# xrouting/xroute_env

Measured on AMD Instinct MI355X. Metric: env-steps/sec (batched regions), ispd18_test1-sized regions, higher is better.
Workload: dtype u32 distances / i16 state / fp32 observation

## Files before the change

xroute_env_amd/csrc/xr_kernels.hip:

```cpp
#include <hip/hip_runtime.h>
#include <stdint.h>
#include <initializer_list>
#include <type_traits>

#include "xr_device.h"
#include "../../include/xroute_hip.h"

#define XR_FNV_PRIME 0x100000001b3ULL

__device__ __forceinline__ void fnv_mix(uint64_t& h, uint32_t w) { h = (h ^ (uint64_t)w) * XR_FNV_PRIME; }

__device__ __forceinline__ uint64_t splitmix64(uint64_t x) {
    x += 0x9E3779B97F4A7C15ULL;
    uint64_t z = x;
    z = (z ^ (z >> 30)) * 0xBF58476D1CE4E5B9ULL;
    z = (z ^ (z >> 27)) * 0x94D049BB133111EBULL;
    return z ^ (z >> 31);
}

__global__ void xr_ingest_kernel(const uint32_t* __restrict__ rec, int16_t* __restrict__ node_net,
                                 int16_t* __restrict__ owner0, int64_t total) {
    int64_t i = (int64_t)blockIdx.x * blockDim.x + threadIdx.x;
    const int64_t stride = (int64_t)gridDim.x * blockDim.x;
    for (; i < total; i += stride) {
// ... 717 lines not shown
    const uint64_t* lw = b.legal + (int64_t)row * b.legal_words;
    int act = 0;
    for (int w = 0; w < b.legal_words; w++) {
        uint64_t m = lw[w];
        const int pc = __popcll(m);
        if (j >= pc) { j -= pc; continue; }
        while (j > 0) { m &= m - 1; j--; }
        act = w * 64 + __ffsll((long long)m);
        break;
    }
    return act;
}

__global__ void xr_random_action_kernel(XrBatchDev b, int32_t* __restrict__ actions, uint64_t seed) {
    const int e = b.env_base + blockIdx.x * blockDim.x + threadIdx.x;
    if (e >= XR_ENV_END(b)) return;
    actions[e] = xr_random_pick(b, e, e, seed);
}

struct XrStateSrc {
    const int16_t* node_net;
    const int16_t* owner;
    __device__ __forceinline__ int net(int f) const { const int n = node_net[f]; return n; }
    __device__ __forceinline__ bool used(int f) const { return owner[f] != 0; }
};
struct XrRecSrc {
    const uint32_t* rec;
    __device__ __forceinline__ int net(int f) const {
        const uint32_t r = rec[f];
        const uint32_t t = XR_REC_TYPE(r);
        return t == XR_TYPE_ACCESS ? (int)XR_REC_NET1(r) : (t == XR_TYPE_BLOCKAGE ? -1 : 0);
    }
    __device__ __forceinline__ bool used(int f) const { return XR_REC_USED(rec[f]) != 0; }
};

template <class Src>
__device__ __forceinline__ void xr_node_features(const Src& s, int f, int X, int Y, int Z, int N, float& obst,
                                                 int& apnet, bool& adj) {
    if (f >= N) { obst = 0.f; apnet = 0; adj = false; return; }
    const int n = s.net(f);
    const bool used = s.used(f);
    obst = (n == -1 || used) ? 1.f : 0.f;
    apnet = n > 0 ? n : 0;
    adj = false;
    if (n > 0) {
        const int z = f % Z, y = (f / Z) % Y, x = f / (Y * Z);
        const int YZ = Y * Z;
        if (x + 1 < X && s.net(f + YZ) == n) adj = true;
        else if (y > 0 && s.net(f - Z) == n) adj = true;
        else if (x > 0 && s.net(f - YZ) == n) adj = true;
        else if (y + 1 < Y && s.net(f + Z) == n) adj = true;
        else if (z + 1 < Z && s.net(f + 1) == n) adj = true;
        else if (z > 0 && s.net(f - 1) == n) adj = true;
    }
}

typedef float xr_f4 __attribute__((ext_vector_type(4)));
#define XR_ST4(ptr, val) __builtin_nontemporal_store(xr_f4{(val).x, (val).y, (val).z, (val).w}, reinterpret_cast<xr_f4*>(ptr))
template <class Src, int VEC>
__device__ __forceinline__ void xr_obs_write(const Src& s, int X, int Y, int Z, int N, const int* s_ids, int K,
                                             float* __restrict__ out, int chunk_base, int knets = -1) {
    if (knets < 0) knets = K;
    const int f0 = chunk_base + threadIdx.x * VEC;
    if (f0 >= N) return;
    float obst[VEC];
    int apnet[VEC];
    bool adj[VEC];
#pragma unroll
    for (int j = 0; j < VEC; j++) xr_node_features(s, f0 + j, X, Y, Z, N, obst[j], apnet[j], adj[j]);
    float* p = out + f0;
    if (VEC == 4) {
        float4 v;
        v.x = obst[0]; v.y = obst[1]; v.z = obst[2]; v.w = obst[3];
        XR_ST4(p, v);
        p += N;
        v.x = (f0 + 0 < K) ? (float)s_ids[f0 + 0] : 0.f;
        v.y = (f0 + 1 < K) ? (float)s_ids[f0 + 1] : 0.f;
        v.z = (f0 + 2 < K) ? (float)s_ids[f0 + 2] : 0.f;
        v.w = (f0 + 3 < K) ? (float)s_ids[f0 + 3] : 0.f;
        XR_ST4(p, v);
        p += N;
        bool anyap = false;
#pragma unroll
        for (int j = 0; j < VEC; j++) anyap |= (apnet[j] != 0);
        const float4 zero = make_float4(0.f, 0.f, 0.f, 0.f);
        for (int i = 0; i < knets; i++) {
            float4 m = zero, ma = zero;
            if (anyap) {
                const int id = s_ids[i];
                m.x = (apnet[0] == id) ? 1.f : 0.f; m.y = (apnet[1] == id) ? 1.f : 0.f;
                m.z = (apnet[2] == id) ? 1.f : 0.f; m.w = (apnet[3] == id) ? 1.f : 0.f;
                ma.x = (adj[0] ? m.x : 0.f); ma.y = (adj[1] ? m.y : 0.f);
                ma.z = (adj[2] ? m.z : 0.f); ma.w = (adj[3] ? m.w : 0.f);
            }
            XR_ST4(p, m);
            p += N;
#pragma unroll
            for (int c = 0; c < 6; c++) { XR_ST4(p, ma); p += N; }
        }
    } else {
        p[0] = obst[0];
        p += N;
        p[0] = (f0 < K) ? (float)s_ids[f0] : 0.f;
        p += N;
        for (int i = 0; i < knets; i++) {
            const float m = (apnet[0] != 0 && apnet[0] == s_ids[i]) ? 1.f : 0.f;
            const float ma = adj[0] ? m : 0.f;
            p[0] = m;
            p += N;
#pragma unroll
            for (int c = 0; c < 6; c++) { p[0] = ma; p += N; }
        }
    }
}

__device__ __forceinline__ float xr_plane_value(unsigned ft, int plane, int node, const int* s_ids, int K) {
    if (plane >= 2) {
        const int pi = plane - 2, i = pi / 7, c = pi - 7 * i;
        const unsigned id = (unsigned)s_ids[i];
        return c ? (((ft & 0x7FFFu) == (id | 0x4000u)) ? 1.f : 0.f) : (((ft & 0x3FFFu) == id) ? 1.f : 0.f);
    }
    if (plane == 0) return (ft & 0x8000u) ? 1.f : 0.f;
    return node < K ? (float)s_ids[node] : 0.f;
}

template <class Src>
__device__ __forceinline__ void xr_obs_env_stream(const Src& src, int X, int Y, int Z, int N, const int* s_ids, int K,
                                                  float* __restrict__ out, unsigned short* s_feat, int planes = -1) {
    const int tid = threadIdx.x, nthr = blockDim.x;
#pragma unroll 4
    for (int f = tid; f < N; f += nthr) {
        float obst; int apnet; bool adj;
        xr_node_features(src, f, X, Y, Z, N, obst, apnet, adj);
        s_feat[f] = (unsigned short)(apnet | (adj ? 0x4000 : 0) | (obst != 0.f ? 0x8000 : 0));
    }
    __syncthreads();
    const long long total = (long long)(planes >= 0 ? planes : 2 + 7 * K) * N;
    const long long nslot = total >> 2;
    int plane = (int)((4LL * tid) / N), node = (int)((4LL * tid) - (long long)plane * N);
    const int dplane = (4 * nthr) / N, dnode = (4 * nthr) - dplane * N;
    for (long long sidx = tid; sidx < nslot; sidx += nthr) {
        float v[4];
        if (node + 3 < N && plane >= 2) {
            const int pi = plane - 2, i = pi / 7, c = pi - 7 * i;
            const unsigned id = (unsigned)s_ids[i];
            const unsigned msk = c ? 0x7FFFu : 0x3FFFu, want = c ? (id | 0x4000u) : id;
#pragma unroll
            for (int j = 0; j < 4; j++) v[j] = ((s_feat[node + j] & msk) == want) ? 1.f : 0.f;
        } else {
            int p = plane, f = node;
#pragma unroll
            for (int j = 0; j < 4; j++) {
                v[j] = xr_plane_value(s_feat[f], p, f, s_ids, K);
                if (++f == N) { f = 0; ++p; }
            }
        }
        XR_ST4(out + 4 * sidx, make_float4(v[0], v[1], v[2], v[3]));
        plane += dplane; node += dnode;
        if (node >= N) { node -= N; ++plane; }
    }
    const int tail = (int)(total & 3);
    if (tid < tail) {
        const long long g = (nslot << 2) + tid;
        const int p = (int)(g / N), f = (int)(g - (long long)p * N);
        out[g] = xr_plane_value(s_feat[f], p, f, s_ids, K);
    }
}

__device__ __forceinline__ int xr_legal_ids_pre(uint64_t my_m, int words, int* s_ids, int* s_pref) {
    const int tid = threadIdx.x;
    if (tid < words) s_pref[tid] = __popcll(my_m);
    xr_lds_barrier();
    if (tid == 0) {
        int acc = 0;
        for (int w = 0; w < words; w++) { const int c = s_pref[w]; s_pref[w] = acc; acc += c; }
        s_pref[words] = acc;
    }
    xr_lds_barrier();
    if (tid < words) {
        uint64_t m = my_m;
        int o = s_pref[tid];
        while (m) { const int bit = __ffsll((long long)m) - 1; s_ids[o++] = tid * 64 + bit + 1; m &= m - 1; }
    }
    xr_lds_barrier();
    return s_pref[words];
}
__device__ __forceinline__ int xr_legal_ids(const uint64_t* __restrict__ lw, int words, int* s_ids, int* s_pref) {
    const int tid = threadIdx.x;
    for (int w = tid; w < words; w += blockDim.x) s_pref[w] = __popcll(lw[w]);
    __syncthreads();
    if (tid == 0) {
        int acc = 0;
        for (int w = 0; w < words; w++) { const int c = s_pref[w]; s_pref[w] = acc; acc += c; }
        s_pref[words] = acc;
    }
    __syncthreads();
    for (int w = tid; w < words; w += blockDim.x) {
        uint64_t m = lw[w];
        int o = s_pref[w];
        while (m) { const int bit = __ffsll((long long)m) - 1; s_ids[o++] = w * 64 + bit + 1; m &= m - 1; }
    }
    __syncthreads();
    return s_pref[words];
}

template <int VEC>
__global__ void xr_obs_kernel(XrBatchDev b, float* __restrict__ out, int64_t env_stride, int env_lo) {
    extern __shared__ __attribute__((aligned(16))) char smem[];
    int* s_ids = reinterpret_cast<int*>(smem);
    int* s_pref = s_ids + b.legal_words * 64;
    const int e = env_lo + blockIdx.y;
    const XrRegionDev R = b.regions[b.env_region[e]];
    const int chunk_base = blockIdx.x * blockDim.x * VEC;
    if (chunk_base >= R.N) return;
    const int K = xr_legal_ids(b.legal + (int64_t)e * b.legal_words, b.legal_words, s_ids, s_pref);
    XrStateSrc src{b.rg_node_net + R.node_off, b.owner + (int64_t)e * b.n_max};
    xr_obs_write<XrStateSrc, VEC>(src, R.X, R.Y, R.Z, R.N, s_ids, K, out + (int64_t)blockIdx.y * env_stride,
                                  chunk_base);
}

__global__ void xr_obs_stream_kernel(XrBatchDev b, float* __restrict__ out, int64_t env_stride, int env_lo) {
    extern __shared__ __attribute__((aligned(16))) char smem[];
    int* s_ids = reinterpret_cast<int*>(smem);
    int* s_pref = s_ids + b.legal_words * 64;
    unsigned short* s_feat = reinterpret_cast<unsigned short*>(s_pref + ((b.legal_words + 1 + 3) & ~3));
    const int e = env_lo + blockIdx.x;
    const XrRegionDev R = b.regions[b.env_region[e]];
    const int K = xr_legal_ids(b.legal + (int64_t)e * b.legal_words, b.legal_words, s_ids, s_pref);
    XrStateSrc src{b.rg_node_net + R.node_off, b.owner + (int64_t)e * b.n_max};
    xr_obs_env_stream(src, R.X, R.Y, R.Z, R.N, s_ids, K, out + (int64_t)blockIdx.x * env_stride, s_feat);
}

template <int VEC>
__global__ void xr_obs_records_kernel(const uint32_t* __restrict__ rec, int X, int Y, int Z,
                                      const int32_t* __restrict__ nets, int K, float* __restrict__ out) {
    extern __shared__ __attribute__((aligned(16))) char smem[];
    int* s_ids = reinterpret_cast<int*>(smem);
    for (int i = threadIdx.x; i < K; i += blockDim.x) s_ids[i] = nets[i];
    __syncthreads();
    XrRecSrc src{rec};
    xr_obs_write<XrRecSrc, VEC>(src, X, Y, Z, X * Y * Z, s_ids, K, out, blockIdx.x * blockDim.x * VEC);
}

__device__ __forceinline__ void xr_obs_epilogue(const XrBatchDev& b, int e, char* smem, bool head_only) {
    __syncthreads();
    const XrRegionDev R = b.regions[b.env_region[e]];
    int* s_ids = reinterpret_cast<int*>(smem);
    int* s_pref = s_ids + b.legal_words * 64;
    XrStateSrc src{b.rg_node_net + R.node_off, b.owner + (int64_t)e * b.n_max};
    float* __restrict__ out = b.obs_out + (int64_t)e * b.obs_stride;
    const int ids_bytes = ((b.legal_words * 64 + b.legal_words + 1) * 4 + 15) & ~15;
    const int npad = (R.N + 7) & ~7;
    if (b.obs_vec4 == 1 && ids_bytes + 4 * npad <= b.obs_lds_bytes && b.legal_words <= (int)blockDim.x) {
        const int tid = threadIdx.x, nthr = (int)blockDim.x;
        const uint64_t my_m = tid < b.legal_words ? b.legal[(int64_t)e * b.legal_words + tid] : 0ull;
        int16_t* l_nn = reinterpret_cast<int16_t*>(smem + ids_bytes);
        int16_t* l_ow = l_nn + npad;
        const int nchunk = npad >> 3;
#pragma unroll 4
        for (int ci = tid; ci < nchunk; ci += nthr) {
            const int4 vn = *reinterpret_cast<const int4*>(src.node_net + (ci << 3));
            const int4 vo = *reinterpret_cast<const int4*>(src.owner + (ci << 3));
            *reinterpret_cast<int4*>(l_nn + (ci << 3)) = vn;
            *reinterpret_cast<int4*>(l_ow + (ci << 3)) = vo;
        }
        const int K = xr_legal_ids_pre(my_m, b.legal_words, s_ids, s_pref);
        const int knets = head_only ? XR_SPLIT_KEEP(b, K) : K;
        XrStateSrc lsrc{l_nn, l_ow};
        for (int cb = 0; cb < R.N; cb += nthr * 4)
            xr_obs_write<XrStateSrc, 4>(lsrc, R.X, R.Y, R.Z, R.N, s_ids, K, out, cb, knets);
        return;
    }
    const int feat_bytes = (b.legal_words * 64 + ((b.legal_words + 1 + 3) & ~3)) * 4;
    if (b.obs_vec4 == 2 && feat_bytes + 4 * npad <= b.obs_lds_bytes && b.legal_words <= (int)blockDim.x) {
        const int tid = threadIdx.x, nthr = (int)blockDim.x;
        const uint64_t my_m = tid < b.legal_words ? b.legal[(int64_t)e * b.legal_words + tid] : 0ull;
        unsigned short* s_feat = reinterpret_cast<unsigned short*>(smem + feat_bytes);
        int16_t* l_nn = reinterpret_cast<int16_t*>(smem + feat_bytes + 2 * npad);
        const int nchunk = npad >> 3;
#pragma unroll 4
        for (int ci = tid; ci < nchunk; ci += nthr)
            *reinterpret_cast<int4*>(l_nn + (ci << 3)) = *reinterpret_cast<const int4*>(src.node_net + (ci << 3));
        const int K = xr_legal_ids_pre(my_m, b.legal_words, s_ids, s_pref);
        XrStateSrc lsrc{l_nn, src.owner};
        const int planes = head_only ? 2 + 7 * XR_SPLIT_KEEP(b, K) : -1;
        xr_obs_env_stream(lsrc, R.X, R.Y, R.Z, R.N, s_ids, K, out, s_feat, planes);
        return;
    }
    const int K = xr_legal_ids(b.legal + (int64_t)e * b.legal_words, b.legal_words, s_ids, s_pref);
    if (b.obs_vec4 == 1) {
        const int knets = head_only ? XR_SPLIT_KEEP(b, K) : K;
        for (int cb = 0; cb < R.N; cb += (int)blockDim.x * 4)
            xr_obs_write<XrStateSrc, 4>(src, R.X, R.Y, R.Z, R.N, s_ids, K, out, cb, knets);
    } else if (b.obs_vec4 == 2) {
        unsigned short* s_feat = reinterpret_cast<unsigned short*>(s_pref + ((b.legal_words + 1 + 3) & ~3));
        const int planes = head_only ? 2 + 7 * XR_SPLIT_KEEP(b, K) : -1;
        xr_obs_env_stream(src, R.X, R.Y, R.Z, R.N, s_ids, K, out, s_feat, planes);
    } else {
        for (int cb = 0; cb < R.N; cb += (int)blockDim.x)
            xr_obs_write<XrStateSrc, 1>(src, R.X, R.Y, R.Z, R.N, s_ids, K, out, cb);
    }
}

__device__ __forceinline__ int xr_route_work_class(const XrBatchDev& b, const int32_t* __restrict__ actions, int e) {
    const int a = actions[e];
    const XrRegionDev& R = b.regions[b.env_region[e]];
    if (a < 1 || a > R.n_nets || b.done[e]) return 0;
    if (!((b.legal[(int64_t)e * b.legal_words + ((a - 1) >> 6)] >> ((a - 1) & 63)) & 1ull)) return 0;
    if (b.net_meas) { const int m = b.net_meas[R.net_off + a]; if (m) return m; }
    return b.net_work[R.net_off + a];
}

__global__ void __launch_bounds__(1024) xr_route_order_kernel(XrBatchDev b, const int32_t* __restrict__ actions, int32_t* __restrict__ order) {
    __shared__ uint32_t s_cnt[256];
    __shared__ uint32_t s_wsum[4];
    const int t = threadIdx.x;
    if (t < 256) s_cnt[t] = 0;
    __syncthreads();
    const int e0 = b.env_base, e1 = XR_ENV_END(b);
    int cls[8];
#pragma unroll
    for (int k = 0; k < 8; k++) {
        const int e = e0 + t + k * 1024;
        cls[k] = e < e1 ? xr_route_work_class(b, actions, e) : -1;
        if (cls[k] >= 0) atomicAdd(&s_cnt[cls[k]], 1u);
    }
    for (int e = e0 + t + 8 * 1024; e < e1; e += 1024) atomicAdd(&s_cnt[xr_route_work_class(b, actions, e)], 1u);
    __syncthreads();
    uint32_t v = 0, incl = 0;
    if (t < 256) {
        v = s_cnt[255 - t];
        incl = v;
        for (int o = 1; o < 64; o <<= 1) {
            const uint32_t u = __shfl_up(incl, o, 64);
            if ((t & 63) >= o) incl += u;
        }
        if ((t & 63) == 63) s_wsum[t >> 6] = incl;
    }
    __syncthreads();
    if (t < 256) {
        uint32_t base = 0;
        for (int w = 0; w < (t >> 6); w++) base += s_wsum[w];
        s_cnt[255 - t] = base + incl - v;
    }
    __syncthreads();
#pragma unroll
    for (int k = 0; k < 8; k++)
        if (cls[k] >= 0) order[atomicAdd(&s_cnt[cls[k]], 1u)] = e0 + t + k * 1024;
    for (int e = e0 + t + 8 * 1024; e < e1; e += 1024) order[atomicAdd(&s_cnt[xr_route_work_class(b, actions, e)], 1u)] = e;
}

template <bool LDS_DIST, int ZCH>
__global__ void __launch_bounds__(1024, 4) xr_route_kernel(XrBatchDev b, const int32_t* __restrict__ actions) {
    extern __shared__ __attribute__((aligned(16))) char smem[];
#ifdef XR_TIMELINE
    if (threadIdx.x == 0) {
        b.phase_cycles[(int64_t)blockIdx.x * 8 + 0] = (long long)wall_clock64();
        b.phase_cycles[(int64_t)blockIdx.x * 8 + 3] = (long long)__smid();
    }
#endif
    const int e_ = b.route_order ? b.route_order[blockIdx.x] : (int)blockIdx.x + b.env_base;
    xr_route_dispatch<LDS_DIST, ZCH>(b, e_, actions[e_], smem);
#ifdef XR_TIMELINE
    if (threadIdx.x == 0) b.phase_cycles[(int64_t)blockIdx.x * 8 + 1] = (long long)wall_clock64();
#endif
    if (b.obs_out) xr_obs_epilogue(b, e_, smem, b.obs_head_only != 0);
#ifdef XR_TIMELINE
    __syncthreads();
    if (threadIdx.x == 0) b.phase_cycles[(int64_t)blockIdx.x * 8 + 2] = (long long)wall_clock64();
#endif
}

template <int BT>
__global__ void __launch_bounds__(BT) xr_plan_kernel(XrBatchDev b, const int32_t* __restrict__ actions, uint32_t* __restrict__ next_queue,
                                                     int32_t* __restrict__ order) {
    __shared__ int s_wsum[BT / 64];
    __shared__ int s_base;
    const int tid = threadIdx.x, lane = tid & 63, wv = tid >> 6;
    const int e = b.env_base + blockIdx.x * BT + tid, e_end = XR_ENV_END(b);
    if (blockIdx.x == 0 && tid < 3 && next_queue) next_queue[tid] = 0u;
    int k = 0, r = 0;
    const uint64_t* lsrc = nullptr;
    int clear_bit = -1;
    bool was_reset = false;
    if (e < e_end) {
        const int nl = b.nlegal[e];
        r = b.env_region[e];
        was_reset = (nl == 0);
        if (nl == 0) {
            if (b.auto_reset) {
                if (b.env_replay[e] == b.max_route_count) r = (int)(((int64_t)r + b.n_envs) % b.n_regions);
                const XrRegionDev R = b.regions[r];
                lsrc = b.legal0 + R.legal0_off;
                k = R.nlegal0;
            }
        } else {
            const XrRegionDev R = b.regions[r];
            const int a = actions[e];
            lsrc = b.legal + (int64_t)e * b.legal_words;
            k = nl;
            if (a >= 1 && a <= R.n_nets && ((lsrc[(a - 1) >> 6] >> ((a - 1) & 63)) & 1ULL)) {
                clear_bit = a - 1;
                k = nl - 1;
            }
        }
        b.plan_region[e] = r;
    }
    int kskip = XR_SPLIT_KEEP(b, k);
    if (b.obs_incremental && e < e_end && !was_reset) {
        if (clear_bit < 0) kskip = k;
        else {
            int below = 0;
            for (int w = 0; w <= (clear_bit >> 6); w++) {
                uint64_t m = lsrc[w];
                if (w == (clear_bit >> 6)) m &= (1ULL << (clear_bit & 63)) - 1ULL;
                below += __popcll(m);
            }
            kskip = below;
        }
    }
    const int kw = k - kskip;
    int incl = kw;
#pragma unroll
    for (int d = 1; d < 64; d <<= 1) {
        const int t = __shfl_up(incl, d, 64);
        if (lane >= d) incl += t;
    }
    if (lane == 63) s_wsum[wv] = incl;
    __syncthreads();
    int woff = 0;
    for (int w = 0; w < wv; w++) woff += s_wsum[w];
    if (tid == BT - 1) s_base = (int)atomicAdd(&b.queue[2], (unsigned)(woff + incl));
    __syncthreads();
    const int off = s_base + woff + incl - kw;
    if (e < e_end) {
        int j = 0;
        for (int w = 0; w < b.legal_words && j < k; w++) {
            uint64_t m = lsrc[w];
            if (clear_bit >= 0 && (clear_bit >> 6) == w) m &= ~(1ULL << (clear_bit & 63));
            while (m) {
                const int bit = __ffsll((unsigned long long)m) - 1;
                m &= m - 1;
                if (j >= kskip) {
                    b.plan_units[off + j - kskip] = ((uint32_t)e << 14) | (uint32_t)j;
                    b.plan_unit_net[off + j - kskip] = (w << 6) + bit + 1;
                }
                j++;
            }
        }
    }
    if (order) {
        __shared__ uint32_t s_cnt[256];
        __shared__ uint32_t s_csum[4];
        if (tid < 256) s_cnt[tid] = 0;
        __syncthreads();
        const int cls = e < e_end ? xr_route_work_class(b, actions, e) : -1;
        if (cls >= 0) atomicAdd(&s_cnt[cls], 1u);
        __syncthreads();
        uint32_t v = 0, inc = 0;
        if (tid < 256) {
            v = s_cnt[255 - tid];
            inc = v;
            for (int o = 1; o < 64; o <<= 1) {
                const uint32_t u = __shfl_up(inc, o, 64);
                if (lane >= o) inc += u;
            }
            if (lane == 63) s_csum[wv] = inc;
        }
        __syncthreads();
        if (tid < 256) {
            uint32_t base = 0;
            for (int w = 0; w < wv; w++) base += s_csum[w];
            s_cnt[255 - tid] = base + inc - v;
        }
        __syncthreads();
        if (cls >= 0) order[atomicAdd(&s_cnt[cls], 1u)] = e;
    }
}

#define XR_NP_J 9
template <int J = XR_NP_J>
__device__ __forceinline__ void xr_unit_aligned(const XrBatchDev& b, int u, int t_lo = 0, int t_hi = 1 << 22) {
    const int tid = threadIdx.x;
    const uint32_t ent = b.plan_units[u];
    const int id = b.plan_unit_net[u];
    const int e = (int)(ent >> 14), rank = (int)(ent & 0x3FFFu);
    const XrRegionDev R = b.regions[b.plan_region[e]];
    const int N = R.N, Z = R.Z, Y = R.Y, X = R.X, YZ = Y * Z;
    const int16_t* __restrict__ nn = b.rg_node_net + R.node_off;
    float* __restrict__ out = b.obs_out + (int64_t)e * b.obs_stride + (int64_t)(2 + 7 * rank) * N;
    const int ngrp = N >> 2;
    const int ap_lo = b.net_csr[R.net_off + id], ap_hi = b.net_csr[R.net_off + id + 1];
    (void)nn; (void)X; (void)Y; (void)Z; (void)YZ;
    const int gend = min(ngrp, t_hi << 8);
    for (int g0 = t_lo << 8; g0 < gend; g0 += 256 * J) {
        unsigned bits[J];
#pragma unroll
        for (int j = 0; j < J; j++) bits[j] = 0;
        for (int i = ap_lo; i < ap_hi; i++) {
            const int v = b.ap_feat[R.ap_off + i];
            const int f = v & 0x7FFFFFFF;
            const unsigned m = (1u | (v < 0 ? 16u : 0u)) << (f & 3);
            const int g = (f >> 2) - g0 - tid;
#pragma unroll
            for (int j = 0; j < J; j++) bits[j] |= (g == j * 256) ? m : 0u;
        }
#pragma unroll
        for (int j = 0; j < J; j++) {
            const int g = g0 + j * 256 + tid;
            if (g < gend) {
                float* __restrict__ pp = out + ((int64_t)g << 2);
                const unsigned m0 = bits[j], m1 = bits[j] >> 4;
                float4 v0, v1;
                v0.x = (m0 & 1u) ? 1.f : 0.f; v0.y = (m0 & 2u) ? 1.f : 0.f; v0.z = (m0 & 4u) ? 1.f : 0.f; v0.w = (m0 & 8u) ? 1.f : 0.f;
                v1.x = (m1 & 1u) ? 1.f : 0.f; v1.y = (m1 & 2u) ? 1.f : 0.f; v1.z = (m1 & 4u) ? 1.f : 0.f; v1.w = (m1 & 8u) ? 1.f : 0.f;
                XR_ST4(pp, v0);
#pragma unroll
                for (int pl = 1; pl < 7; pl++) XR_ST4(pp + (int64_t)pl * N, v1);
            }
        }
    }
}

__global__ void __launch_bounds__(256) xr_netplane_kernel(XrBatchDev b) {
    const int total = (int)b.queue[2];
    for (int u = blockIdx.x; u < total; u += gridDim.x) xr_unit_aligned(b, u);
}

__device__ __forceinline__ void xr_unit_stream(const XrBatchDev& b, int u, uint32_t* s_m) {
    const int tid = threadIdx.x;
    const uint32_t ent = b.plan_units[u];
    const int id = b.plan_unit_net[u];
    const int e = (int)(ent >> 14), rank = (int)(ent & 0x3FFFu);
    const XrRegionDev R = b.regions[b.plan_region[e]];
    const int N = R.N, Z = R.Z, Y = R.Y, X = R.X, YZ = Y * Z;
    const int nwords = (N + 15) >> 4;
    (void)X; (void)Y; (void)Z; (void)YZ;
    const int ap_lo = b.net_csr[R.net_off + id], ap_hi = b.net_csr[R.net_off + id + 1];
    int my_ap = 0;
    const bool has_ap = ap_lo + tid < ap_hi;
    if (has_ap) my_ap = b.ap_feat[R.ap_off + ap_lo + tid];
    for (int w = tid; w <= nwords; w += 256) s_m[w] = 0u;
    xr_lds_barrier();
    if (has_ap) {
        const int f = my_ap & 0x7FFFFFFF;
        atomicOr(&s_m[f >> 4], (my_ap < 0 ? 3u : 1u) << ((f & 15) << 1));
    }
    xr_lds_barrier();
    float* __restrict__ run = b.obs_out + (int64_t)e * b.obs_stride + (int64_t)(2 + 7 * rank) * N;
    const int total = 7 * N;
    const int head = (int)((32u - (uint32_t)((reinterpret_cast<uintptr_t>(run) >> 2) & 31u)) & 31u);
    const int nslot = total > head ? (total - head) >> 2 : 0;
    const int piece = ((nslot + 7 * 256 - 1) / (7 * 256)) * 256;
    auto one = [&](int o) -> float {
        int pl = 0, f = o;
        while (f >= N) { f -= N; pl++; }
        return ((s_m[f >> 4] >> (((f & 15) << 1) + (pl ? 1 : 0))) & 1u) ? 1.f : 0.f;
    };
    int ppl[7], pnd[7];
#pragma unroll
    for (int p = 0; p < 7; p++) {
        int o = head + ((p * piece + tid) << 2), pl = 0;
        while (o >= N && pl < 7) { o -= N; pl++; }
        ppl[p] = pl; pnd[p] = o;
    }
    for (int it = 0; it < piece; it += 256) {
#pragma unroll
        for (int p = 0; p < 7; p++) {
            const int sl = p * piece + it + tid;
            if (sl < nslot) {
                const int f = pnd[p], pl = ppl[p];
                float4 v;
                if (f + 3 < N) {
                    const int bit = f << 1, w = bit >> 5;
                    const uint32_t m = __funnelshift_r(s_m[w], s_m[w + 1], bit & 31) >> (pl ? 1 : 0);
                    v.x = (m & 1u) ? 1.f : 0.f; v.y = (m & 4u) ? 1.f : 0.f; v.z = (m & 16u) ? 1.f : 0.f; v.w = (m & 64u) ? 1.f : 0.f;
                } else {
                    const int o = head + (sl << 2);
                    v.x = one(o); v.y = one(o + 1); v.z = one(o + 2); v.w = one(o + 3);
                }
                XR_ST4(run + head + (sl << 2), v);
            }
            int nf = pnd[p] + 1024;
            while (nf >= N) { nf -= N; ppl[p]++; }
            pnd[p] = nf;
        }
    }
    if (tid < head && tid < total) run[tid] = one(tid);
    const int tail0 = head + (nslot << 2);
    if (tid >= 64 && tail0 + (tid - 64) < total) run[tail0 + (tid - 64)] = one(tail0 + (tid - 64));
    xr_lds_barrier();
}

typedef unsigned xr_u4 __attribute__((ext_vector_type(4)));
#define XR_STU8(ptr, v) __builtin_nontemporal_store((v), reinterpret_cast<xr_u4*>(ptr))
__device__ __forceinline__ uint32_t xr_nib_bytes(uint32_t m) {
    return (m & 1u) | ((m & 2u) << 7) | ((m & 4u) << 14) | ((m & 8u) << 21);
}
__device__ __forceinline__ xr_u4 xr_bits_bytes16(uint32_t m) {
    return xr_u4{xr_nib_bytes(m), xr_nib_bytes(m >> 4), xr_nib_bytes(m >> 8), xr_nib_bytes(m >> 12)};
}
__device__ __forceinline__ uint32_t xr_pair_bytes(uint32_t m) {
    return (m & 1u) | ((m & 4u) << 6) | ((m & 16u) << 12) | ((m & 64u) << 18);
}
__device__ __forceinline__ uint32_t xr_obst_bytes4(uint32_t n0, uint32_t n1, uint32_t w0, uint32_t w1) {
    auto ob = [](uint32_t n, uint32_t w) -> uint32_t { return ((n & 0xFFFFu) == 0xFFFFu || (w & 0xFFFFu) != 0u) ? 1u : 0u; };
    return ob(n0, w0) | (ob(n0 >> 16, w0 >> 16) << 8) | (ob(n1, w1) << 16) | (ob(n1 >> 16, w1 >> 16) << 24);
}

__device__ __forceinline__ void xr_obs_head_u8(const XrBatchDev& b, int e, char* smem) {
    __syncthreads();
    const XrRegionDev R = b.regions[b.env_region[e]];
    int* s_ids = reinterpret_cast<int*>(smem);
    int* s_pref = s_ids + b.legal_words * 64;
    const int tid = threadIdx.x, nthr = (int)blockDim.x;
    int K;
    if (b.legal_words <= nthr) {
        const uint64_t my_m = tid < b.legal_words ? b.legal[(int64_t)e * b.legal_words + tid] : 0ull;
        K = xr_legal_ids_pre(my_m, b.legal_words, s_ids, s_pref);
    } else {
        K = xr_legal_ids(b.legal + (int64_t)e * b.legal_words, b.legal_words, s_ids, s_pref);
    }
    const int16_t* __restrict__ nn = b.rg_node_net + R.node_off;
    const int16_t* __restrict__ ow = b.owner + (int64_t)e * b.n_max;
    uint8_t* __restrict__ out = b.obs_out_u8 + (int64_t)e * b.obs_stride;
    const int N = R.N, total = 2 * N, nslot = total >> 4;
    auto one = [&](int o) -> uint32_t {
        if (o < N) return (nn[o] == -1 || ow[o] != 0) ? 1u : 0u;
        return o - N < K ? ((uint32_t)s_ids[o - N] & 0xFFu) : 0u;
    };
    for (int s = tid; s < nslot; s += nthr) {
        const int o = s << 4;
        xr_u4 v;
        if (o + 16 <= N) {
            const int4 a0 = *reinterpret_cast<const int4*>(nn + o), a1 = *reinterpret_cast<const int4*>(nn + o + 8);
            const int4 c0 = *reinterpret_cast<const int4*>(ow + o), c1 = *reinterpret_cast<const int4*>(ow + o + 8);
            v = xr_u4{xr_obst_bytes4(a0.x, a0.y, c0.x, c0.y), xr_obst_bytes4(a0.z, a0.w, c0.z, c0.w),
                      xr_obst_bytes4(a1.x, a1.y, c1.x, c1.y), xr_obst_bytes4(a1.z, a1.w, c1.z, c1.w)};
        } else if (o >= N + K) {
            v = xr_u4{0u, 0u, 0u, 0u};
        } else {
            uint32_t w[4];
#pragma unroll
            for (int q = 0; q < 4; q++)
                w[q] = one(o + 4 * q) | (one(o + 4 * q + 1) << 8) | (one(o + 4 * q + 2) << 16) | (one(o + 4 * q + 3) << 24);
            v = xr_u4{w[0], w[1], w[2], w[3]};
        }
        XR_STU8(out + o, v);
    }
    const int tail0 = nslot << 4;
    if (tid < total - tail0) out[tail0 + tid] = (uint8_t)one(tail0 + tid);
}

#define XR_NPU8_J 4
__device__ __forceinline__ void xr_unit_u8_aligned(const XrBatchDev& b, int u) {
    const int tid = threadIdx.x, nthr = (int)blockDim.x;
    const uint32_t ent = b.plan_units[u];
    const int id = b.plan_unit_net[u];
    const int e = (int)(ent >> 14), rank = (int)(ent & 0x3FFFu);
    const XrRegionDev R = b.regions[b.plan_region[e]];
    const int N = R.N;
    uint8_t* __restrict__ out = b.obs_out_u8 + (int64_t)e * b.obs_stride + (int64_t)(2 + 7 * rank) * N;
    const int ngrp = N >> 4;
    const int ap_lo = b.net_csr[R.net_off + id], ap_hi = b.net_csr[R.net_off + id + 1];
    for (int g0 = 0; g0 < ngrp; g0 += nthr * XR_NPU8_J) {
        uint32_t bits[XR_NPU8_J];
#pragma unroll
        for (int j = 0; j < XR_NPU8_J; j++) bits[j] = 0;
        for (int i = ap_lo; i < ap_hi; i++) {
            const int v = b.ap_feat[R.ap_off + i];
            const int f = v & 0x7FFFFFFF;
            const uint32_t m = (1u | (v < 0 ? 0x10000u : 0u)) << (f & 15);
            const int g = (f >> 4) - g0 - tid;
#pragma unroll
            for (int j = 0; j < XR_NPU8_J; j++) bits[j] |= (g == j * nthr) ? m : 0u;
        }
#pragma unroll
        for (int j = 0; j < XR_NPU8_J; j++) {
            const int g = g0 + j * nthr + tid;
            if (g < ngrp) {
                uint8_t* __restrict__ pp = out + ((int64_t)g << 4);
                const xr_u4 v0 = xr_bits_bytes16(bits[j]), v1 = xr_bits_bytes16(bits[j] >> 16);
                XR_STU8(pp, v0);
#pragma unroll
                for (int pl = 1; pl < 7; pl++) XR_STU8(pp + (int64_t)pl * N, v1);
            }
        }
    }
}

__device__ __forceinline__ void xr_unit_u8_stream(const XrBatchDev& b, int u, uint32_t* s_m) {
    const int tid = threadIdx.x, nthr = (int)blockDim.x;
    const uint32_t ent = b.plan_units[u];
    const int id = b.plan_unit_net[u];
    const int e = (int)(ent >> 14), rank = (int)(ent & 0x3FFFu);
    const XrRegionDev R = b.regions[b.plan_region[e]];
    const int N = R.N;
    const int nwords = (N + 15) >> 4;
    const int ap_lo = b.net_csr[R.net_off + id], ap_hi = b.net_csr[R.net_off + id + 1];
    for (int w = tid; w <= nwords; w += nthr) s_m[w] = 0u;
    xr_lds_barrier();
    for (int i = ap_lo + tid; i < ap_hi; i += nthr) {
        const int v = b.ap_feat[R.ap_off + i];
        const int f = v & 0x7FFFFFFF;
        atomicOr(&s_m[f >> 4], (v < 0 ? 3u : 1u) << ((f & 15) << 1));
    }
    xr_lds_barrier();
    uint8_t* __restrict__ run = b.obs_out_u8 + (int64_t)e * b.obs_stride + (int64_t)(2 + 7 * rank) * N;
    const int total = 7 * N;
    const int head = min(total, (int)((128u - (uint32_t)(reinterpret_cast<uintptr_t>(run) & 127u)) & 127u));
    const int nslot = (total - head) >> 4;
    auto one = [&](int o) -> uint32_t {
        const int pl = o / N, f = o - pl * N;
        return (s_m[f >> 4] >> (((f & 15) << 1) + (pl ? 1 : 0))) & 1u;
    };
    for (int sl = tid; sl < nslot; sl += nthr) {
        const int o = head + (sl << 4);
        const int pl = o / N, f = o - pl * N;
        xr_u4 v;
        if (f + 15 < N) {
            const int bit = f << 1, w = bit >> 5;
            const uint32_t m = __funnelshift_r(s_m[w], s_m[w + 1], bit & 31) >> (pl ? 1 : 0);
            v = xr_u4{xr_pair_bytes(m), xr_pair_bytes(m >> 8), xr_pair_bytes(m >> 16), xr_pair_bytes(m >> 24)};
        } else {
            uint32_t q4[4];
#pragma unroll
            for (int q = 0; q < 4; q++)
                q4[q] = one(o + 4 * q) | (one(o + 4 * q + 1) << 8) | (one(o + 4 * q + 2) << 16) | (one(o + 4 * q + 3) << 24);
            v = xr_u4{q4[0], q4[1], q4[2], q4[3]};
        }
        XR_STU8(run + o, v);
    }
    for (int i = tid; i < head; i += nthr) run[i] = (uint8_t)one(i);
    const int tail0 = head + (nslot << 4);
    for (int i = tail0 + tid; i < total; i += nthr) run[i] = (uint8_t)one(i);
    xr_lds_barrier();
}

__global__ void __launch_bounds__(256) xr_obs_u8_kernel(XrBatchDev b, uint8_t* __restrict__ out, int64_t env_stride, int env_lo) {
    extern __shared__ __attribute__((aligned(16))) char smem[];
    int* s_ids = reinterpret_cast<int*>(smem);
    int* s_pref = s_ids + b.legal_words * 64;
    const int e = env_lo + blockIdx.y;
    const XrRegionDev R = b.regions[b.env_region[e]];
    const int N = R.N;
    const int64_t slot0 = (int64_t)blockIdx.x * blockDim.x;
    if ((slot0 << 4) >= (int64_t)(2 + 7 * (int64_t)R.n_nets) * N) return;
    const int K = xr_legal_ids(b.legal + (int64_t)e * b.legal_words, b.legal_words, s_ids, s_pref);
    const int64_t total = (int64_t)(2 + 7 * (int64_t)K) * N;
    const int64_t o = (slot0 + threadIdx.x) << 4;
    if (o >= total) return;
    XrStateSrc src{b.rg_node_net + R.node_off, b.owner + (int64_t)e * b.n_max};
    uint8_t* __restrict__ row = out + (int64_t)blockIdx.y * env_stride;
    int p = (int)(o / N), f = (int)(o - (int64_t)p * N);
    uint32_t w[4] = {0u, 0u, 0u, 0u};
    const int cnt = total - o < 16 ? (int)(total - o) : 16;
    for (int j = 0; j < cnt; j++) {
        float obst; int apnet; bool adj;
        xr_node_features(src, f, R.X, R.Y, R.Z, N, obst, apnet, adj);
        uint32_t v;
        if (p == 0) v = obst != 0.f ? 1u : 0u;
        else if (p == 1) v = f < K ? ((uint32_t)s_ids[f] & 0xFFu) : 0u;
        else {
            const int pi = p - 2, i = pi / 7, c = pi - 7 * i;
            v = (apnet != 0 && apnet == s_ids[i] && (c == 0 || adj)) ? 1u : 0u;
        }
        w[j >> 2] |= v << ((j & 3) << 3);
        if (++f == N) { f = 0; ++p; }
    }
    if (cnt == 16) {
        XR_STU8(row + o, (xr_u4{w[0], w[1], w[2], w[3]}));
    } else {
        for (int j = 0; j < cnt; j++) row[o + j] = (uint8_t)(w[j >> 2] >> ((j & 3) << 3));
    }
}

constexpr int XR_QUEUE_BATCH = 1;
constexpr int XR_TICKET_TILES = 3;
static_assert(XR_TICKET_TILES >= 1 && XR_TICKET_TILES <= XR_NP_J, "a slab is one pass of xr_unit_aligned");
__device__ __forceinline__ void xr_queue_first(int G, int sh, int& first_r, int& first_u) {
// ... 663 lines not shown
```

Baseline: 2.340 million.

## Use per-wave class ranking and register-cached legal masks in plan/order kernels

The route-order and plan kernels now build per-wave class histograms. Each lane's slot within its class is found with an LDS atomicOr bitmask and popcount, instead of one LDS atomicAdd per env on a shared block-wide counter. The plan kernel merges the class ordering into its existing pass, which removes the separate barrier-heavy scan section. It also keeps up to four legal-mask words in registers and skips a barrier when only one block is launched. The aim is less LDS atomic contention and fewer barriers and global reloads, at the cost of much more LDS use and a rank step that relies on implicit wave-lockstep visibility.

```diff
diff --git a/xroute_env_amd/csrc/xr_kernels.hip b/xroute_env_amd/csrc/xr_kernels.hip
--- a/xroute_env_amd/csrc/xr_kernels.hip
+++ b/xroute_env_amd/csrc/xr_kernels.hip
@@ -1043,52 +1043,103 @@
     }
 }
 
+__device__ __forceinline__ int xr_net_work_class(const XrBatchDev& b, int idx) {
+    const int w = b.net_work[idx];
+    const int m = b.net_meas ? b.net_meas[idx] : 0;
+    return m ? m : w;
+}
+
 __device__ __forceinline__ int xr_route_work_class(const XrBatchDev& b, const int32_t* __restrict__ actions, int e) {
     const int a = actions[e];
-    const XrRegionDev& R = b.regions[b.env_region[e]];
-    if (a < 1 || a > R.n_nets || b.done[e]) return 0;
-    if (!((b.legal[(int64_t)e * b.legal_words + ((a - 1) >> 6)] >> ((a - 1) & 63)) & 1ull)) return 0;
-    if (b.net_meas) { const int m = b.net_meas[R.net_off + a]; if (m) return m; }
-    return b.net_work[R.net_off + a];
+    const int r = b.env_region[e];
+    const int dn = b.done[e];
+    const bool in_words = a >= 1 && a <= b.legal_words * 64;
+    const uint64_t m = b.legal[(int64_t)e * b.legal_words + (in_words ? (a - 1) >> 6 : 0)];
+    const int net_off = b.regions[r].net_off;
+    if (!in_words || dn || !((m >> ((a - 1) & 63)) & 1ull)) return 0;
+    return xr_net_work_class(b, net_off + a);
+}
+
+__device__ __forceinline__ void xr_wave_class_rank(int cls, int lane, unsigned long long* cm, int& rank, int& cnt, bool& first) {
+    unsigned long long same = 0;
+    if (cls >= 0) atomicOr(&cm[cls], 1ULL << lane);
+    if (cls >= 0) same = *reinterpret_cast<volatile unsigned long long*>(&cm[cls]);
+    if (cls >= 0) *reinterpret_cast<volatile unsigned long long*>(&cm[cls]) = 0ULL;
+    rank = __popcll(same & ((1ULL << lane) - 1ULL));
+    cnt = __popcll(same);
+    first = cls >= 0 && rank == 0;
+}
+
+template <int NW>
+__device__ __forceinline__ void xr_class_wave_scan(uint32_t* s_wc, uint32_t* s_csum, int tid) {
+    const int lane = tid & 63, wv = tid >> 6;
+    uint32_t v = 0, inc = 0;
+    if (tid < 256) {
+        for (int w = 0; w < NW; w++) v += s_wc[w * 256 + 255 - tid];
+        inc = v;
+        for (int o = 1; o < 64; o <<= 1) {
+            const uint32_t u = __shfl_up(inc, o, 64);
+            if (lane >= o) inc += u;
+        }
+        if (lane == 63) s_csum[wv] = inc;
+    }
+    __syncthreads();
+    if (tid < 256) {
+        uint32_t run = inc - v;
+        for (int w = 0; w < wv; w++) run += s_csum[w];
+        for (int w = 0; w < NW; w++) {
+            const uint32_t c = s_wc[w * 256 + 255 - tid];
+            s_wc[w * 256 + 255 - tid] = run;
+            run += c;
+        }
+    }
+    __syncthreads();
 }
 
 __global__ void __launch_bounds__(1024) xr_route_order_kernel(XrBatchDev b, const int32_t* __restrict__ actions, int32_t* __restrict__ order) {
-    __shared__ uint32_t s_cnt[256];
-    __shared__ uint32_t s_wsum[4];
-    const int t = threadIdx.x;
-    if (t < 256) s_cnt[t] = 0;
+    __shared__ uint32_t s_wc[16 * 256];
+    __shared__ uint32_t s_csum[4];
+    const int t = threadIdx.x, lane = t & 63, wv = t >> 6;
+    __shared__ unsigned long long s_cm[16 * 256];
+    volatile uint32_t* const row = s_wc + wv * 256;
+    unsigned long long* const cm = s_cm + wv * 256;
+#pragma unroll
+    for (int i = 0; i < 4; i++) {
+        row[lane + 64 * i] = 0;
+        cm[lane + 64 * i] = 0ULL;
+    }
+    const int e0 = b.env_base, e1 = XR_ENV_END(b);
+    const int per = (((e1 - e0 + 15) >> 4) + 63) & ~63;
+    const int w0 = e0 + wv * per, w1 = min(e1, w0 + per);
+    int cls[8];
+#pragma unroll
+    for (int k = 0; k < 8; k++) {
+        const int e = w0 + k * 64 + lane;
+        cls[k] = e < w1 ? xr_route_work_class(b, actions, e) : -1;
+    }
+#pragma unroll
+    for (int k = 0; k < 8; k++)
+        if (cls[k] >= 0) atomicAdd(&s_wc[wv * 256 + cls[k]], 1u);
+    for (int e = w0 + 8 * 64 + lane; e < w1; e += 64) atomicAdd(&s_wc[wv * 256 + xr_route_work_class(b, actions, e)], 1u);
     __syncthreads();
-    const int e0 = b.env_base, e1 = XR_ENV_END(b);
-    int cls[8];
+    xr_class_wave_scan<16>(s_wc, s_csum, t);
 #pragma unroll
     for (int k = 0; k < 8; k++) {
-        const int e = e0 + t + k * 1024;
-        cls[k] = e < e1 ? xr_route_work_class(b, actions, e) : -1;
-        if (cls[k] >= 0) atomicAdd(&s_cnt[cls[k]], 1u);
-    }
-    for (int e = e0 + t + 8 * 1024; e < e1; e += 1024) atomicAdd(&s_cnt[xr_route_work_class(b, actions, e)], 1u);
-    __syncthreads();
-    uint32_t v = 0, incl = 0;
-    if (t < 256) {
-        v = s_cnt[255 - t];
-        incl = v;
-        for (int o = 1; o < 64; o <<= 1) {
-            const uint32_t u = __shfl_up(incl, o, 64);
-            if ((t & 63) >= o) incl += u;
-        }
-        if ((t & 63) == 63) s_wsum[t >> 6] = incl;
-    }
-    __syncthreads();
-    if (t < 256) {
-        uint32_t base = 0;
-        for (int w = 0; w < (t >> 6); w++) base += s_wsum[w];
-        s_cnt[255 - t] = base + incl - v;
-    }
-    __syncthreads();
-#pragma unroll
-    for (int k = 0; k < 8; k++)
-        if (cls[k] >= 0) order[atomicAdd(&s_cnt[cls[k]], 1u)] = e0 + t + k * 1024;
-    for (int e = e0 + t + 8 * 1024; e < e1; e += 1024) order[atomicAdd(&s_cnt[xr_route_work_class(b, actions, e)], 1u)] = e;
+        int rank, cnt;
+        bool first;
+        xr_wave_class_rank(cls[k], lane, cm, rank, cnt, first);
+        if (cls[k] >= 0) order[row[cls[k]] + rank] = w0 + k * 64 + lane;
+        if (first) row[cls[k]] += cnt;
+    }
+    for (int eb = w0 + 8 * 64; eb < w1; eb += 64) {
+        const int e = eb + lane;
+        const int c = e < w1 ? xr_route_work_class(b, actions, e) : -1;
+        int rank, cnt;
+        bool first;
+        xr_wave_class_rank(c, lane, cm, rank, cnt, first);
+        if (c >= 0) order[row[c] + rank] = e;
+        if (first) row[c] += cnt;
+    }
 }
 
 template <bool LDS_DIST, int ZCH>
@@ -1115,50 +1166,108 @@
 template <int BT>
 __global__ void __launch_bounds__(BT) xr_plan_kernel(XrBatchDev b, const int32_t* __restrict__ actions, uint32_t* __restrict__ next_queue,
                                                      int32_t* __restrict__ order) {
-    __shared__ int s_wsum[BT / 64];
+    constexpr int NW = BT / 64;
+    constexpr bool CAN_ORDER = BT == 1024;
+    __shared__ int s_wsum[NW];
     __shared__ int s_base;
+    __shared__ uint32_t s_wc[CAN_ORDER ? NW * 256 : 1];
+    __shared__ uint32_t s_csum[4];
+    __shared__ unsigned long long s_cm[CAN_ORDER ? NW * 256 : 1];
     const int tid = threadIdx.x, lane = tid & 63, wv = tid >> 6;
     const int e = b.env_base + blockIdx.x * BT + tid, e_end = XR_ENV_END(b);
-    if (blockIdx.x == 0 && tid < 3 && next_queue) next_queue[tid] = 0u;
-    int k = 0, r = 0;
-    const uint64_t* lsrc = nullptr;
+    const bool live = e < e_end;
+    const bool ordered = CAN_ORDER && order != nullptr;
+    const int lw = b.legal_words;
+    const bool in_regs = lw <= 4;
+    const uint64_t* const lrow = b.legal + (int64_t)e * lw;
+    int r = 0, a = 0, nl = 0, rep = 0, dn = 0;
+    uint64_t m0 = 0, m1 = 0, m2 = 0, m3 = 0;
+    if (live) {
+        r = b.env_region[e];
+        a = actions[e];
+        nl = b.nlegal[e];
+        rep = b.env_replay[e];
+        if (ordered) dn = b.done[e];
+        if (in_regs) {
+            if (lw > 0) m0 = lrow[0];
+            if (lw > 1) m1 = lrow[1];
+            if (lw > 2) m2 = lrow[2];
+            if (lw > 3) m3 = lrow[3];
+        }
+    }
+    if (CAN_ORDER && ordered) {
+#pragma unroll
+        for (int i = 0; i < 4; i++) {
+            s_wc[wv * 256 + lane + 64 * i] = 0;
+            s_cm[wv * 256 + lane + 64 * i] = 0ULL;
+        }
+    }
+    const int net_off = CAN_ORDER && ordered && live ? b.regions[r].net_off : 0;
+    const bool in_words = a >= 1 && a <= lw * 64;
+    const int ai = in_words ? a - 1 : 0;
+    uint64_t aword;
+    if (in_regs) aword = (ai >> 6) == 0 ? m0 : (ai >> 6) == 1 ? m1 : (ai >> 6) == 2 ? m2 : m3;
+    else aword = live && in_words ? lrow[ai >> 6] : 0;
+    const bool a_legal = live && in_words && ((aword >> (ai & 63)) & 1ULL);
+    int cls = -1;
+    if (CAN_ORDER && ordered && live) cls = a_legal && !dn ? xr_net_work_class(b, net_off + a) : 0;
+    int k = 0;
+    const uint64_t* lsrc = lrow;
     int clear_bit = -1;
-    bool was_reset = false;
-    if (e < e_end) {
-        const int nl = b.nlegal[e];
-        r = b.env_region[e];
-        was_reset = (nl == 0);
+    const bool was_reset = live && nl == 0;
+    if (live) {
         if (nl == 0) {
+            m0 = m1 = m2 = m3 = 0;
+            lsrc = nullptr;
             if (b.auto_reset) {
-                if (b.env_replay[e] == b.max_route_count) r = (int)(((int64_t)r + b.n_envs) % b.n_regions);
-                const XrRegionDev R = b.regions[r];
-                lsrc = b.legal0 + R.legal0_off;
-                k = R.nlegal0;
+                if (rep == b.max_route_count) r = (int)(((int64_t)r + b.n_envs) % b.n_regions);
+                const XrRegionDev* const Rn = b.regions + r;
+                const int64_t l0 = Rn->legal0_off;
+                k = Rn->nlegal0;
+                lsrc = b.legal0 + l0;
+                if (in_regs) {
+                    if (lw > 0) m0 = lsrc[0];
+                    if (lw > 1) m1 = lsrc[1];
+                    if (lw > 2) m2 = lsrc[2];
+                    if (lw > 3) m3 = lsrc[3];
+                }
             }
         } else {
-            const XrRegionDev R = b.regions[r];
-            const int a = actions[e];
-            lsrc = b.legal + (int64_t)e * b.legal_words;
             k = nl;
-            if (a >= 1 && a <= R.n_nets && ((lsrc[(a - 1) >> 6] >> ((a - 1) & 63)) & 1ULL)) {
-                clear_bit = a - 1;
+            if (a_legal) {
+                clear_bit = ai;
                 k = nl - 1;
             }
         }
-        b.plan_region[e] = r;
     }
     int kskip = XR_SPLIT_KEEP(b, k);
-    if (b.obs_incremental && e < e_end && !was_reset) {
+    const int cw = clear_bit >> 6;
+    if (b.obs_incremental && live && !was_reset) {
         if (clear_bit < 0) kskip = k;
         else {
+            const uint64_t low = (1ULL << (clear_bit & 63)) - 1ULL;
             int below = 0;
-            for (int w = 0; w <= (clear_bit >> 6); w++) {
-                uint64_t m = lsrc[w];
-                if (w == (clear_bit >> 6)) m &= (1ULL << (clear_bit & 63)) - 1ULL;
-                below += __popcll(m);
+            if (in_regs) {
+                below = __popcll(cw == 0 ? m0 & low : m0);
+                if (cw >= 1) below += __popcll(cw == 1 ? m1 & low : m1);
+                if (cw >= 2) below += __popcll(cw == 2 ? m2 & low : m2);
+                if (cw >= 3) below += __popcll(m3 & low);
+            } else {
+                for (int w = 0; w <= cw; w++) {
+                    uint64_t m = lsrc[w];
+                    if (w == cw) m &= low;
+                    below += __popcll(m);
+                }
             }
             kskip = below;
         }
+    }
+    if (clear_bit >= 0) {
+        const uint64_t keep = ~(1ULL << (clear_bit & 63));
+        if (cw == 0) m0 &= keep;
+        else if (cw == 1) m1 &= keep;
+        else if (cw == 2) m2 &= keep;
+        else if (cw == 3) m3 &= keep;
     }
     const int kw = k - kskip;
     int incl = kw;
@@ -1168,17 +1277,29 @@
         if (lane >= d) incl += t;
     }
     if (lane == 63) s_wsum[wv] = incl;
+    int crank = 0;
+    if (CAN_ORDER && ordered) {
+        int ccnt;
+        bool cfirst;
+        xr_wave_class_rank(cls, lane, s_cm + wv * 256, crank, ccnt, cfirst);
+        if (cfirst) s_wc[wv * 256 + cls] = (uint32_t)ccnt;
+    }
     __syncthreads();
     int woff = 0;
     for (int w = 0; w < wv; w++) woff += s_wsum[w];
-    if (tid == BT - 1) s_base = (int)atomicAdd(&b.queue[2], (unsigned)(woff + incl));
-    __syncthreads();
-    const int off = s_base + woff + incl - kw;
-    if (e < e_end) {
+    int base = 0;
+    if (gridDim.x == 1) {
+        if (tid == BT - 1) atomicAdd(&b.queue[2], (unsigned)(woff + incl));
+    } else {
+        if (tid == BT - 1) s_base = (int)atomicAdd(&b.queue[2], (unsigned)(woff + incl));
+        __syncthreads();
+        base = s_base;
+    }
+    if (CAN_ORDER && ordered) xr_class_wave_scan<NW>(s_wc, s_csum, tid);
+    const int off = base + woff + incl - kw;
+    if (live) {
         int j = 0;
-        for (int w = 0; w < b.legal_words && j < k; w++) {
-            uint64_t m = lsrc[w];
-            if (clear_bit >= 0 && (clear_bit >> 6) == w) m &= ~(1ULL << (clear_bit & 63));
+        auto emit = [&](uint64_t m, int w) {
             while (m) {
                 const int bit = __ffsll((unsigned long long)m) - 1;
                 m &= m - 1;
@@ -1188,35 +1309,23 @@
                 }
                 j++;
             }
-        }
-    }
-    if (order) {
-        __shared__ uint32_t s_cnt[256];
-        __shared__ uint32_t s_csum[4];
-        if (tid < 256) s_cnt[tid] = 0;
-        __syncthreads();
-        const int cls = e < e_end ? xr_route_work_class(b, actions, e) : -1;
-        if (cls >= 0) atomicAdd(&s_cnt[cls], 1u);
-        __syncthreads();
-        uint32_t v = 0, inc = 0;
-        if (tid < 256) {
-            v = s_cnt[255 - tid];
-            inc = v;
-            for (int o = 1; o < 64; o <<= 1) {
-                const uint32_t u = __shfl_up(inc, o, 64);
-                if (lane >= o) inc += u;
-            }
-            if (lane == 63) s_csum[wv] = inc;
-        }
-        __syncthreads();
-        if (tid < 256) {
-            uint32_t base = 0;
-            for (int w = 0; w < wv; w++) base += s_csum[w];
-            s_cnt[255 - tid] = base + inc - v;
-        }
-        __syncthreads();
-        if (cls >= 0) order[atomicAdd(&s_cnt[cls], 1u)] = e;
-    }
+        };
+        if (in_regs) {
+            if (j < k) emit(m0, 0);
+            if (j < k) emit(m1, 1);
+            if (j < k) emit(m2, 2);
+            if (j < k) emit(m3, 3);
+        } else {
+            for (int w = 0; w < lw && j < k; w++) {
+                uint64_t m = lsrc[w];
+                if (cw == w) m &= ~(1ULL << (clear_bit & 63));
+                emit(m, w);
+            }
+        }
+        b.plan_region[e] = r;
+        if (CAN_ORDER && ordered) order[s_wc[wv * 256 + cls] + (uint32_t)crank] = e;
+    }
+    if (blockIdx.x == 0 && tid < 3 && next_queue) next_queue[tid] = 0u;
 }
 
 #define XR_NP_J 9
```

Result: no change. 2.345 million (median of 2 runs) (+0.2%).
